# MacPhobos/audio-ident

Measured on AMD Instinct MI355X. Metric: audio-seconds fingerprinted/sec/GPU; landmark-hash bit-exact vs CPU ref, higher is better.
Workload: dtype f32; 1 GPU; BASELINE configs[1]: 256 x 10 s 44.1 kHz mono clips, fingerprint extraction per GPU; clips_per_gpu=256, n_fft=2048, hop=512, parallelism=clip-sharded x1 (no data-path collective)

## Files before the change

audio-ident_amd/csrc/aidfp_extract.h:

```cpp
#pragma once
#include "aidfp_buffers.h"
#include "aidfp_extract_plan.h"

namespace aid {

struct Extractor {
    DevBuf<float> pcm_stage, power;
    DevBuf<uint64_t> mask, hotw;
    DevBuf<uint32_t> clip_qmax;
    DevBuf<uint32_t> k2_cold;
    HostBuf<uint64_t> h_cold;
    uint64_t *h_cold_dev = nullptr;
    DevBuf<int64_t> chunk_counts, counts;
    DevBuf<uint64_t> records;
    DevBuf<ClipDesc> desc;
    HostBuf<ClipDesc> h_desc;
    size_t desc_n = 0;
    ClipDesc *desc_dev = nullptr;
    Event desc_ev, stage_ev;
    hipStream_t stage_stream = nullptr;
    K2Policy k2;
    int64_t k2_slots[2] = {1, 1};
    int64_t k1_slots = 1;
    int64_t plane_rows = 0;
    ExtractPlan plan;
    bool have_result = false;
};

}
```

audio-ident_amd/csrc/aidfp_extract_plan.h:

```cpp
#pragma once
#include <string.h>

#include <algorithm>
#include <vector>

#include "../../include/aidfp.h"
#include "aidfp_layout.h"

namespace aid {

constexpr int64_t kPlaneRows = (int64_t)3 << 18;
constexpr int kK2Hold = 64;

struct K2Choice {
    int width;
    double slots_x;
};

struct K2Policy {
    int width = 4;
    int hold = 0;
    int force_width = 0;
    double force_slots_x = 0.0;

    K2Choice choose(uint64_t cw, uint64_t sw) {
        const int seen_width = (sw >> 32) ? (int)((cw >> 32) / (sw >> 32)) : 0;
        if (force_width) {
            width = force_width;
        } else if (width == 4) {
            if (hold > 0) --hold;
            else if (seen_width == 4 && 2 * (uint64_t)(uint32_t)cw >= (cw >> 32)) width = 2;
        } else if (seen_width == 2 && (uint32_t)sw > 0) {
            width = 4;
            hold = kK2Hold;
        }
        if (force_slots_x > 0.0) return {width, force_slots_x};
        if (width != 4 || seen_width != 4) return {width, 1.0};
        const double c = std::min(1.0, (double)(uint32_t)cw / (double)(cw >> 32));
        return {width, c >= 0.45 ? 1.5 : c >= 0.3 ? 1.25 : 1.0};
    }
};

struct ClipGroup {
    int first = 0, n = 0;
    int64_t frame0 = 0, frames = 0;
    int64_t strips = 0, k1_strips = 0;
    int strip_len = 0;
};

struct ExtractPlan {
    std::vector<ClipDesc> desc;
    std::vector<int64_t> frames, hash_base;
    std::vector<ClipGroup> groups;
    int n_clips = 0, width = 4;
    int64_t total_frames = 0, strips = 0, chunks = 0, records = 0;
    int64_t staged = 0;
    bool empty_clip = false;
    bool multi_chunk = false, one_chunk_each = false;
};

inline void plan_extract(ExtractPlan &p, const int64_t *offsets, const int64_t *ends, int n_clips, int loc, int hop,
                         int64_t plane_rows, bool keep_power, int64_t slots, double slots_x, int width) {
    auto clip_end = [&](int c) { return ends ? ends[c] : offsets[c + 1]; };
    p.n_clips = n_clips;
    p.width = width;
    p.desc.resize(n_clips);
    p.frames.resize(n_clips);
    p.hash_base.resize(n_clips);
    p.groups.clear();
    const int64_t cap = plane_rows > 0 ? plane_rows : kPlaneRows;
    int first = 0;
    int64_t acc = 0;
    for (int c = 0; c < n_clips; ++c) {
        p.frames[c] = num_frames(clip_end(c) - offsets[c], hop);
        if (!keep_power && acc > 0 && acc + p.frames[c] > cap) {
            p.groups.push_back({first, c - first});
            first = c;
            acc = 0;
        }
        acc += p.frames[c];
    }
    p.groups.push_back({first, n_clips - first});
    p.total_frames = p.strips = p.chunks = p.records = 0;
    p.staged = loc == AID_PCM_HOST && n_clips > 0 ? clip_end(n_clips - 1) - offsets[0] : 0;
    p.empty_clip = p.multi_chunk = false;
    p.one_chunk_each = n_clips > 0;
    int64_t k1_strips = 0;
    for (ClipGroup &g : p.groups) {
        g.strip_len = peak_strip_len(p.frames.data() + g.first, g.n, std::max<int64_t>(1, (int64_t)(slots * slots_x)));
        g.frame0 = p.total_frames;
        for (int c = g.first; c < g.first + g.n; ++c) {
            const int64_t F = p.frames[c], nck = (F + kHashChunk - 1) / kHashChunk;
            p.desc[c] = {loc == AID_PCM_DEVICE ? offsets[c] : offsets[c] - offsets[0], F, p.total_frames, g.strips,
                         p.chunks, p.records, hash_capacity(F), k1_strips};
            p.hash_base[c] = p.records;
            p.empty_clip |= F == 0;
            p.multi_chunk |= nck > 1;
            p.one_chunk_each &= nck == 1;
            p.total_frames += F;
            g.frames += F;
            g.strips += (F + g.strip_len - 1) / g.strip_len;
            g.k1_strips += (F + kStftStrip - 1) / kStftStrip;
            k1_strips += (F + kStftStrip - 1) / kStftStrip;
            p.chunks += nck;
            p.records += hash_capacity(F);
        }
        p.strips += g.strips;
    }
}

inline bool desc_differ(const ClipDesc *a, size_t na, const ClipDesc *b, size_t nb) {
    return na != nb || (na > 0 && memcmp(a, b, na * sizeof(ClipDesc)) != 0);
}

}
```

audio-ident_amd/csrc/aidfp_launch.h:

```cpp
#pragma once
#include <hip/hip_runtime.h>
#include <stdint.h>

#include "aidfp_device.h"

namespace aid {
void launch_stft_power(const void *pcm, bool s16, const ClipDesc *clips, int n_clips, int64_t f0, int64_t total_frames,
                       int64_t total_strips, int64_t slots, int hop, const Tables *tab, float *out, bool logmag,
                       uint64_t *hot, float thr, bool keep_power, uint32_t *qmax, hipStream_t s);
int peak_pick_blocks_per_cu(int width);
void launch_peak_pick(int width, const float *power, const ClipDesc *clips, int n_clips, int64_t f0, int64_t total_strips,
                      int strip_len, float thr, const uint64_t *hot, uint64_t *mask, uint32_t *cold_cnt,
                      const uint32_t *clip_qmax, float rel, hipStream_t s);
void launch_landmarks(const uint64_t *mask, const ClipDesc *clips, int n_clips, int64_t total_chunks,
                      int64_t *chunk_counts, uint64_t *records, int64_t *clip_counts, bool write, uint32_t *k2_cold,
                      uint64_t *k2_cold_host, uint32_t k2_waves, uint32_t k2_strips, bool one_chunk_each,
                      hipStream_t s);
void launch_synth(float *out, const uint32_t *tracks, const int64_t *starts, int n_clips, int64_t n, int sr,
                  int noise_a, uint32_t salt, int fmax_hz, bool envelope, const int16_t *sin_tab, hipStream_t s);
void launch_resample(const void *src, bool s16, int64_t in_base, int64_t n, int channels, int up, int down, int hl,
                     int J, const float *taps, float *dst, int64_t m_first, int64_t count, hipStream_t s,
                     int n_streams = 1, int64_t src_stride = 0, int64_t dst_stride = 0, const void *hist = nullptr,
                     int64_t hist_n = 0, int64_t hist_stride = 0);
struct SpeedVarDev;
void launch_resample_speeds(const void *src, bool s16, int channels, const int64_t *clip_off, const SpeedVarDev *vars,
                            int n_speeds, const int64_t *blk_first, const int64_t *dst_off, int pair0, int n_pairs,
                            int64_t blocks, int64_t lds_floats, float *dst, hipStream_t s);
void launch_s16_to_f32(const int16_t *src, int64_t n, float *dst, hipStream_t s);
int dedup_chunks(int64_t n_cat);
void launch_dedup_scan(const uint32_t *cw, const int64_t *coff, const double *cdur, int64_t n_cat, const uint32_t *qw,
                       const int64_t *qoff, const double *qlo, const double *qhi, int nq, double *part_sim,
                       int64_t *part_idx, double *best_sim, int64_t *best_idx, hipStream_t s);
void launch_dedup_pairs(const uint32_t *aw, const int64_t *aoff, const uint32_t *bw, const int64_t *boff, int n,
                        double *sim, hipStream_t s);
void launch_index_count(const uint32_t *ph, const uint32_t *ptrack, int64_t n, const uint8_t *tomb, uint32_t n_tracks,
                        uint32_t *cnt, hipStream_t s);
void launch_index_scatter(const uint32_t *ph, const uint32_t *ptrack, const uint32_t *pt, int64_t n,
                          const uint8_t *tomb, uint32_t n_tracks, uint32_t *cursor, uint64_t *post, hipStream_t s);
void launch_scan(const uint32_t *in, uint32_t *out, int64_t n, uint32_t *tmp, hipStream_t s);
int match_lds_blocks_per_cu();
size_t radix_scratch_u32(int64_t n);
hipError_t launch_index_sort_build(const uint32_t *ph, const uint32_t *ptrack, const uint32_t *pt, int64_t n,
                                   const uint8_t *tomb, uint32_t n_tracks, uint32_t *keys0, uint32_t *keys1,
                                   uint64_t *vals0, uint64_t *vals1, uint32_t *scratch, uint32_t *E, uint32_t *offsets,
                                   unsigned long long *nz, uint64_t **vals_out, uint16_t *sig, int rank_mode,
                                   hipStream_t s);
void launch_make_sig(const uint64_t *post, int64_t n, uint16_t *sig, hipStream_t s);
void launch_compact(const uint32_t *ph, const uint32_t *ptrack, const uint32_t *pt, int64_t n, const uint8_t *tomb,
                    uint32_t n_tracks, uint32_t *cnt, uint32_t *off, uint32_t *tmp, uint32_t *oh, uint32_t *otrack,
                    uint32_t *ot, hipStream_t s);
// ... 45 lines not shown
```

audio-ident_amd/csrc/aidfp_layout.h:

```cpp
#pragma once
#include <stdint.h>

namespace aid {

constexpr int kN = 2048;
constexpr int kBins = 1024;
constexpr int kPeakDT = 7;
constexpr int kPeakDF = 15;
constexpr int kZoneDT = 63;
constexpr int kZoneDF = 127;
constexpr int kFan = 10;
constexpr int kMaskWords = kBins / 64;

constexpr int kStftWaves = 16;
constexpr int kStftStrip = 16;
constexpr int kK1MinFrames = 2;
constexpr int kStftLdsPerWave = 1092;

constexpr int kPeakStripMin = 16;
constexpr int kPeakStripMax = 65536;

inline int peak_strip_len(const int64_t *frames, int n, int64_t slots) {
    int64_t fmax = 0;
    for (int c = 0; c < n; ++c) fmax = frames[c] > fmax ? frames[c] : fmax;
// ... 2 lines not shown
        for (int c = 0; c < n; ++c) k += (frames[c] + L - 1) / L;
        return k;
    };
    int64_t lo = kPeakStripMin, hi = fmax > lo ? fmax : lo;
    if (hi > kPeakStripMax) hi = kPeakStripMax;
    if (count(lo) <= slots) return (int)lo;
    while (lo < hi) {
        const int64_t mid = (lo + hi) / 2;
        if (count(mid) <= slots) hi = mid; else lo = mid + 1;
    }
    return (int)lo;
}

constexpr int hot_bit(int c) { return c < 32 ? c : 95 - c; }

__host__ __device__ constexpr uint32_t bucket_key(uint32_t h) {
    return (((h >> 22) & 0xFFu) << 18) | ((h >> 30) << 16) | (((h >> 12) & 0x7Fu) << 9) | (((h >> 19) & 0x7u) << 6) |
           (h & 0x3Fu);
}

__host__ __device__ constexpr uint16_t posting_sig(uint32_t track, uint32_t t) {
    return (uint16_t)(((track * 0x9E3779B1u) >> 16) + t);
}

constexpr int64_t kLdsMaxVotes = (int64_t)1 << 18;

constexpr int kHashChunk = 1024;
constexpr int kHashChunkPeakCap = 64 * ((kHashChunk + kZoneDT + 7) / 8);

inline int64_t num_frames(int64_t n, int hop) { return (hop <= 0 || n < kN) ? 0 : 1 + (n - kN) / hop; }
inline int64_t peak_capacity(int64_t F) { return 64 * ((F + 7) / 8); }
inline int64_t hash_capacity(int64_t F) { return kFan * peak_capacity(F); }

struct ClipDesc {
    int64_t pcm_off;
    int64_t frames;
    int64_t frame_base;
    int64_t strip_base;
    int64_t chunk_base;
    int64_t hash_base;
    int64_t hash_cap;
    int64_t stft_base;
};

}
```

audio-ident_amd/csrc/extract.cpp:

```cpp
#include <cstring>

#include "engine_internal.h"

int extract_locked(aid_engine *e, const void *pcm, PcmFmt fmt, const int64_t *offsets, int32_t n_clips, int32_t loc,
                   void *stream, const int64_t *ends) {
    if (ends && loc != AID_PCM_DEVICE) return fail(AID_ERR_INVALID, "extract: clip ends need device PCM");
    HIP_TRY(hipSetDevice(e->device));
    Extractor &x = e->ext;
    ExtractPlan &p = x.plan;
    hipStream_t s = pick_stream(e, stream);
    const bool keep_power = (e->cfg.flags & AID_FLAG_KEEP_POWER) != 0, rel = e->cfg.peak_rel > 0.0f;
    if (e->last_stream && e->last_stream != s) HIP_TRY(hipStreamSynchronize(e->last_stream));
    x.have_result = false;
    const uint64_t cw = x.h_cold.p ? *reinterpret_cast<volatile uint64_t *>(x.h_cold.p) : 0;
    const uint64_t sw = x.h_cold.p ? *reinterpret_cast<volatile uint64_t *>(x.h_cold.p + 1) : 0;
    const K2Choice k2 = x.k2.choose(cw, sw);
    plan_extract(p, offsets, ends, n_clips, loc, e->cfg.hop, x.plane_rows, keep_power,
                 x.k2_slots[k2.width == 2 ? 0 : 1], k2.slots_x, k2.width);
    int64_t plane = 1;
    for (const ClipGroup &g : p.groups) plane = std::max(plane, g.frames);
    HIP_TRY(x.desc.reserve((size_t)n_clips + 1));
    HIP_TRY(x.power.reserve((size_t)plane * kBins));
    HIP_TRY(x.mask.reserve((size_t)p.total_frames * kMaskWords));
    HIP_TRY(x.hotw.reserve((size_t)p.total_frames + 1));
    if (rel) {
        HIP_TRY(x.clip_qmax.reserve((size_t)n_clips + 1));
        if (n_clips > 0) HIP_TRY(hipMemsetAsync(x.clip_qmax.p, 0, sizeof(uint32_t) * (size_t)n_clips, s));
    }
    if (!x.h_cold.p) {
        HIP_TRY(x.k2_cold.reserve(128));
        HIP_TRY(hipMemsetAsync(x.k2_cold.p, 0, 128 * sizeof(uint32_t), s));
        HIP_TRY(x.h_cold.reserve(2, hipHostMallocMapped));
        x.h_cold.p[0] = x.h_cold.p[1] = 0;
        HIP_TRY(hipHostGetDevicePointer((void **)&x.h_cold_dev, x.h_cold.p, 0));
    }
    HIP_TRY(x.chunk_counts.reserve((size_t)p.chunks + 1));
    HIP_TRY(x.records.reserve((size_t)p.records + 1));
    HIP_TRY(x.counts.reserve((size_t)n_clips + 1));
    const void *dpcm = pcm;
    if (p.staged > 0) {
        if (x.stage_stream != s) HIP_TRY(x.stage_ev.wait());
        x.stage_ev.live = false;
        const size_t nbytes = (size_t)p.staged * pcm_size(fmt);
        HIP_TRY(x.pcm_stage.reserve((nbytes + sizeof(float) - 1) / sizeof(float)));
        HIP_TRY(hipMemcpyAsync(x.pcm_stage.p, pcm_at(pcm, fmt, offsets[0]), nbytes, hipMemcpyHostToDevice, s));
        dpcm = x.pcm_stage.p;
    }
    if (n_clips > 0 && (x.desc_dev != x.desc.p || desc_differ(p.desc.data(), (size_t)n_clips, x.h_desc.p, x.desc_n))) {
        x.desc_dev = nullptr;
        HIP_TRY(x.desc_ev.wait());
        HIP_TRY(x.h_desc.reserve((size_t)n_clips + 1));
        std::memcpy(x.h_desc.p, p.desc.data(), sizeof(ClipDesc) * n_clips);
        HIP_TRY(hipMemcpyAsync(x.desc.p, x.h_desc.p, sizeof(ClipDesc) * n_clips, hipMemcpyHostToDevice, s));
        HIP_TRY(x.desc_ev.record(s));
        x.desc_n = (size_t)n_clips;
        x.desc_dev = x.desc.p;
    }
    if (p.empty_clip || p.total_frames == 0)
        HIP_TRY(hipMemsetAsync(x.counts.p, 0, sizeof(int64_t) * ((size_t)n_clips + 1), s));
    if (p.total_frames > 0) {
        for (const ClipGroup &g : p.groups) {
            if (g.frames == 0) continue;
            uint32_t *qmax = rel ? x.clip_qmax.p + g.first : nullptr;
            {
                ProfScope ps(e, AID_K_STFT, s, true);
                launch_stft_power(dpcm, fmt == kS16, x.desc.p + g.first, g.n, g.frame0, g.frames, g.k1_strips,
                                  x.k1_slots, e->cfg.hop, e->d_tab.p, x.power.p, false, x.hotw.p,
                                  e->cfg.peak_threshold, keep_power, qmax, s);
            }
            if (loc == AID_PCM_HOST && &g == &p.groups.back()) {
                HIP_TRY(x.stage_ev.record(s));
                x.stage_stream = s;
            }
            {
                ProfScope ps(e, AID_K_PEAKS, s, true);
                launch_peak_pick(p.width, x.power.p, x.desc.p + g.first, g.n, g.frame0, g.strips, g.strip_len,
                                 e->cfg.peak_threshold, x.hotw.p, x.mask.p, x.k2_cold.p, qmax, e->cfg.peak_rel, s);
            }
        }
        if (p.multi_chunk) {
            ProfScope ps(e, AID_K_LANDMARK_COUNT, s, true);
            launch_landmarks(x.mask.p, x.desc.p, n_clips, p.chunks, x.chunk_counts.p, x.records.p, x.counts.p, false,
                             nullptr, nullptr, 0u, 0u, p.one_chunk_each, s);
        }
        {
            ProfScope ps(e, AID_K_LANDMARK_WRITE, s, true);
            launch_landmarks(x.mask.p, x.desc.p, n_clips, p.chunks, x.chunk_counts.p, x.records.p, x.counts.p, true,
                             x.h_cold_dev ? x.k2_cold.p : nullptr, x.h_cold_dev, (uint32_t)(p.width * p.strips),
                             (uint32_t)p.strips, p.one_chunk_each, s);
        }
    }
    HIP_TRY(hipGetLastError());
    e->last_stream = s;
    x.have_result = true;
    return AID_OK;
}

static int result_ready(aid_engine *e, const int32_t *clip, bool wait = true) {
    if (!e) return fail(AID_ERR_INVALID, "null engine");
    if (!e->ext.have_result) return fail(AID_ERR_STATE, "no extraction yet");
    if (clip && (*clip < 0 || *clip >= e->ext.plan.n_clips)) return fail(AID_ERR_INVALID, "clip index out of range");
    return wait ? aid_sync(e) : AID_OK;
}

template <typename T>
static int read_rows(aid_engine *e, int32_t clip, const T *plane, int per, T *out, int64_t cap) {
    const ClipDesc &d = e->ext.plan.desc[clip];
    if (d.frames * per > cap) return fail(AID_ERR_INVALID, "output capacity too small");
    if (d.frames > 0)
        HIP_TRY(hipMemcpy(out, plane + d.frame_base * per, d.frames * per * sizeof(T), hipMemcpyDeviceToHost));
    return AID_OK;
}

extern "C" {

int64_t aid_num_frames(const aid_engine *e, int64_t n) { return e ? num_frames(n, e->cfg.hop) : 0; }
int64_t aid_hash_capacity(const aid_engine *e, int64_t n) { return e ? hash_capacity(num_frames(n, e->cfg.hop)) : 0; }

static int extract_entry(const char *fn, aid_engine *e, const void *pcm, PcmFmt fmt, const int64_t *offsets,
                         int32_t n_clips, int32_t loc, void *stream) {
    if (int rc = check_clips(fn, e, pcm, offsets, n_clips, loc)) return rc;
    std::lock_guard<std::mutex> lk(e->mu);
// ... 44 lines not shown
    if (counts_dev) *counts_dev = e->ext.counts.p;
    if (clip_base_host) *clip_base_host = e->ext.plan.hash_base.data();
    if (n_clips) *n_clips = e->ext.plan.n_clips;
    return AID_OK;
}

int aid_result_power(aid_engine *e, int32_t clip, float *out, int64_t cap) {
    if (int rc = result_ready(e, &clip)) return rc;
    if (!(e->cfg.flags & AID_FLAG_KEEP_POWER))
        return fail(AID_ERR_STATE, "aid_result_power: engine created without AID_FLAG_KEEP_POWER (cold blocks not stored)");
    if (int rc = read_rows(e, clip, e->ext.power.p, kBins, out, cap)) return rc;
    for (int64_t i = 0; i < e->ext.plan.frames[clip] * kBins; ++i) out[i] = out[i] * 0.25f;
    return AID_OK;
}

int aid_result_thresholds(aid_engine *e, float *out) {
    if (int rc = result_ready(e, nullptr)) return rc;
    const int n = e->ext.plan.n_clips;
    if (n > 0 && !out) return fail(AID_ERR_INVALID, "null argument");
    const float thr = e->cfg.peak_threshold, r = e->cfg.peak_rel;
    std::vector<uint32_t> q((size_t)n, 0u);
    if (r > 0.0f && n > 0) HIP_TRY(hipMemcpy(q.data(), e->ext.clip_qmax.p, sizeof(uint32_t) * n, hipMemcpyDeviceToHost));
    for (int c = 0; c < n; ++c) {
        float qm;
        std::memcpy(&qm, &q[c], sizeof(qm));
        const float t = r * (qm * 0.25f);
        out[c] = t > thr ? t : thr;
    }
    return AID_OK;
}

int aid_result_peakmask(aid_engine *e, int32_t clip, uint64_t *out, int64_t cap) {
    if (int rc = result_ready(e, &clip)) return rc;
    return read_rows(e, clip, e->ext.mask.p, kMaskWords, out, cap);
}

int aid_spectrogram(aid_engine *e, const float *pcm, int64_t n, float *out, int64_t cap) {
    if (!e || (n > 0 && !pcm) || n < 0) return fail(AID_ERR_INVALID, "aid_spectrogram: bad argument");
    const int64_t F = num_frames(n, e->cfg.hop);
    if (F * kBins > cap) return fail(AID_ERR_INVALID, "output capacity too small");
    if (F == 0) return AID_OK;
    EngineCall call(e, nullptr, false, kDrainLast);
    if (call.rc) return call.rc;
    hipStream_t s = call.s;
    DevBuf<float> d_pcm, d_out;
    DevBuf<ClipDesc> d_desc;
    ClipDesc d{};
    d.frames = F;
    HIP_TRY(d_pcm.reserve((size_t)n));
    hipError_t he = d_out.reserve((size_t)(F * kBins));
    if (he == hipSuccess) he = d_desc.reserve(1);
    if (he == hipSuccess) he = hipMemcpy(d_pcm.p, pcm, n * sizeof(float), hipMemcpyHostToDevice);
    if (he == hipSuccess) he = hipMemcpy(d_desc.p, &d, sizeof(ClipDesc), hipMemcpyHostToDevice);
    if (he == hipSuccess)
        launch_stft_power(d_pcm.p, false, d_desc.p, 1, 0, F, (F + kStftStrip - 1) / kStftStrip, e->ext.k1_slots,
                          e->cfg.hop, e->d_tab.p, d_out.p, true, nullptr, e->cfg.peak_threshold, true, nullptr, s);
    if (he == hipSuccess) he = hipGetLastError();
    if (he == hipSuccess) he = hipStreamSynchronize(s);
    if (he == hipSuccess) he = hipMemcpy(out, d_out.p, F * kBins * sizeof(float), hipMemcpyDeviceToHost);
    return he == hipSuccess ? AID_OK : fail(AID_ERR_DEVICE, std::string("aid_spectrogram: ") + hipGetErrorString(he));
}

}
```

audio-ident_amd/csrc/landmarks.hip:

```cpp
#include "aidfp_device.h"
#include "aidfp_launch.h"

namespace aid {

constexpr int kK3 = 512;

__device__ __forceinline__ int64_t block_excl_scan(int64_t v, int64_t *tmp , int64_t *total) {
    const int tid = threadIdx.x, lane = tid & 63, w = tid >> 6;
    int64_t x = v;
#pragma unroll
    for (int off = 1; off < 64; off <<= 1) {
        const int64_t y = __shfl_up(x, off, 64);
        if (lane >= off) x += y;
    }
    if (lane == 63) tmp[w] = x;
    __syncthreads();
    int64_t base = 0, tot = 0;
#pragma unroll
    for (int i = 0; i < kK3 / 64; ++i) {
        const int64_t t = tmp[i];
        base += i < w ? t : 0;
        tot += t;
    }
    if (total) *total = tot;
    __syncthreads();
    return base + x - v;
}

__device__ __forceinline__ uint32_t make_hash(int k1, int k2, int dt) {
    return ((uint32_t)(k1 & 0x3FF) << 22) | ((uint32_t)(k2 & 0x3FF) << 12) | ((uint32_t)dt & 0xFFF);
}

template <bool WRITE>
__global__ __launch_bounds__(kK3) void k_landmarks(const uint64_t *__restrict__ mask, const ClipDesc *__restrict__ clips,
                                                  int n_clips, int64_t total_chunks, int64_t *__restrict__ chunk_counts,
                                                  uint64_t *__restrict__ records, int64_t *__restrict__ clip_counts,
                                                  uint32_t *__restrict__ k2_cold, uint64_t *__restrict__ k2_cold_host,
                                                  uint32_t k2_waves, uint32_t k2_strips, int one_chunk_each) {
    __shared__ uint32_t plist[kHashChunkPeakCap];
    __shared__ uint32_t foff[kHashChunk + kZoneDT + 2];
    __shared__ int64_t scan_tmp[kK3];
    const int tid = threadIdx.x;
    const int64_t chunk = blockIdx.x;
    if (WRITE && k2_cold && blockIdx.x == 0 && tid < 64) {
        uint32_t c = k2_cold[tid], c2 = k2_cold[64 + tid];
        k2_cold[tid] = 0u;
        k2_cold[64 + tid] = 0u;
        for (int o = 32; o > 0; o >>= 1) {
            c += __shfl_xor(c, o);
            c2 += __shfl_xor(c2, o);
        }
        if (tid == 0) {
            volatile uint64_t *h = reinterpret_cast<volatile uint64_t *>(k2_cold_host);
            h[0] = (uint64_t)c | ((uint64_t)k2_waves << 32);
            h[1] = (uint64_t)c2 | ((uint64_t)k2_strips << 32);
        }
    }
    if (chunk >= total_chunks) return;
    int lo = 0, hi = n_clips - 1;
    if (one_chunk_each) lo = (int)chunk;
    while (lo < hi) {
        const int mid = (lo + hi + 1) >> 1;
        if (clips[mid].chunk_base <= chunk) lo = mid; else hi = mid - 1;
    }
    const ClipDesc cd = clips[lo];
    const int64_t F = cd.frames;
    const int64_t q = chunk - cd.chunk_base;
    const int64_t c0 = q * kHashChunk;
    const int64_t c1 = min(c0 + (int64_t)kHashChunk, F);
    const int64_t g1 = min(c1 + (int64_t)kZoneDT, F);
    const int nf = (int)(g1 - c0);
    const uint64_t *Mc = mask + (cd.frame_base + c0) * kMaskWords;
    const int64_t nck = (F + kHashChunk - 1) / kHashChunk;
    if (!WRITE && nck == 1) return;

    const int per = (nf + kK3 - 1) / kK3;
    const int fa = min(tid * per, nf), fz = min(fa + per, nf);
    int64_t mine = 0;
    for (int f = fa; f < fz; ++f) {
        uint32_t c = 0;
#pragma unroll
        for (int w = 0; w < kMaskWords; ++w) c += __popcll(Mc[f * kMaskWords + w]);
        foff[f] = c;
        mine += c;
    }
    int64_t npk = 0;
    int64_t run = block_excl_scan(mine, scan_tmp, &npk);
    for (int f = fa; f < fz; ++f) {
        const uint32_t c = foff[f];
        foff[f] = (uint32_t)run;
        if (c == 0) continue;
        int64_t idx = run;
        uint64_t W[kMaskWords];
#pragma unroll
        for (int w = 0; w < kMaskWords; ++w) W[w] = Mc[f * kMaskWords + w];
#pragma unroll
        for (int b = 0; b < 4; ++b) {
            const uint64_t w1 = W[4 * b + 1], w2 = W[4 * b + 2], w3 = W[4 * b + 3];
            for (uint64_t m = W[4 * b] | w1 | w2 | w3; m; m &= m - 1) {
                const int l = __ffsll((unsigned long long)m) - 1;
                const int i = (int)((w1 >> l) & 1) + 2 * (int)((w2 >> l) & 1) + 3 * (int)((w3 >> l) & 1);
                plist[idx++] = ((uint32_t)f << 10) | (uint32_t)(256 * b + 4 * l + i);
            }
        }
        run += c;
    }
    if (tid == 0) foff[nf] = (uint32_t)npk;
    __syncthreads();
    const int n_anchor = (int)foff[c1 - c0];

    const int pa_per = (n_anchor + kK3 - 1) / kK3;
    const int aa = min(tid * pa_per, n_anchor), az = min(aa + pa_per, n_anchor);
    int64_t my = 0;
    uint64_t tmask = 0;
    bool tmask_ok = false;
    for (int i = aa; i < az; ++i) {
        const uint32_t a = plist[i];
        const int ta = (int)(a >> 10), ka = (int)(a & 1023);
        int got = 0;
        uint64_t mk = 0;
        bool ok = true;
        for (int j = i + 1; j < (int)npk && got < kFan; ++j) {
            const uint32_t b = plist[j];
            const int dt = (int)(b >> 10) - ta;
            if (dt > kZoneDT) break;
            if (dt <= 0) continue;
            const int df = (int)(b & 1023) - ka;
            if (df < -kZoneDF || df > kZoneDF) continue;
            if (j - i - 1 < 64) mk |= 1ull << (j - i - 1);
            else ok = false;
            ++got;
        }
// ... 22 lines not shown
                block_excl_scan(all, scan_tmp, &tot);
                if (tid == 0) clip_counts[lo] = tot;
            }
        }
        uint64_t *out = records + cd.hash_base + before + excl;
        int64_t o = 0;
        for (int i = aa; i < az; ++i) {
            const uint32_t a = plist[i];
            const int ta = (int)(a >> 10), ka = (int)(a & 1023);
            const uint64_t t1 = (uint64_t)(c0 + ta) << 32;
            if (i == aa && tmask_ok) {
                for (uint64_t m = tmask; m; m &= m - 1) {
                    const uint32_t b = plist[i + 1 + (__ffsll((unsigned long long)m) - 1)];
                    out[o++] = t1 | make_hash(ka, (int)(b & 1023), (int)(b >> 10) - ta);
                }
                continue;
            }
            int got = 0;
            for (int j = i + 1; j < (int)npk && got < kFan; ++j) {
                const uint32_t b = plist[j];
                const int dt = (int)(b >> 10) - ta;
                if (dt > kZoneDT) break;
                if (dt <= 0) continue;
                const int kb = (int)(b & 1023);
                const int df = kb - ka;
                if (df < -kZoneDF || df > kZoneDF) continue;
                out[o++] = t1 | make_hash(ka, kb, dt);
                ++got;
            }
        }
    }
}

void launch_landmarks(const uint64_t *mask, const ClipDesc *clips, int n_clips, int64_t total_chunks,
                      int64_t *chunk_counts, uint64_t *records, int64_t *clip_counts, bool write, uint32_t *k2_cold,
                      uint64_t *k2_cold_host, uint32_t k2_waves, uint32_t k2_strips, bool one_chunk_each,
                      hipStream_t s) {
    if (total_chunks <= 0) return;
    if (write)
        timed_launch(k_landmarks<true>, dim3((unsigned)total_chunks), dim3(kK3), 0, s, mask, clips, n_clips,
                           total_chunks, chunk_counts, records, clip_counts, k2_cold, k2_cold_host, k2_waves,
                     k2_strips, one_chunk_each ? 1 : 0);
    else
        timed_launch(k_landmarks<false>, dim3((unsigned)total_chunks), dim3(kK3), 0, s, mask, clips, n_clips,
                           total_chunks, chunk_counts, records, clip_counts, (uint32_t *)nullptr, (uint64_t *)nullptr, 0u,
                     0u, one_chunk_each ? 1 : 0);
}

}
```

audio-ident_amd/csrc/peaks.hip:

```cpp
#include "aidfp_device.h"
#include "aidfp_launch.h"

namespace aid {

constexpr int kRowsPerStep = 4;

#if defined(AID_K2_STAMPS)
__device__ unsigned long long g_k2_stamps[8];
#define AID_K2_T() ((unsigned long long)__builtin_amdgcn_s_memtime())
#endif

template <int LANE>
__device__ __forceinline__ uint32_t write_lane(uint32_t v, uint32_t s_val) {
    asm volatile("v_writelane_b32 %0, %1, %2" : "+v"(v) : "s"(s_val), "i"(LANE));
    return v;
}

__device__ __forceinline__ int pkey(float x) {
    float r;
    asm("v_max_f32 %0, 0, %1" : "=v"(r) : "v"(x));
    return __float_as_int(r);
}

struct PeakPickArgs {
    const float *power;
    const ClipDesc *clips;
    int n_clips;
    int64_t f0, total_strips;
    int strip_len;
    float thr;
    const uint64_t *hot;
    uint64_t *mask;
    uint32_t *cold_cnt;
    const uint32_t *clip_qmax;
    float rel;
};

template <int W>
#if defined(AID_K2_PF2) && defined(AID_K2_OCC3)
__global__ __launch_bounds__(64 * W, 3) void k_peak_pick(
#else
__global__ __launch_bounds__(64 * W, 4) void k_peak_pick(
#endif
                                                  const float *__restrict__ power_, const ClipDesc *__restrict__ clips_,
                                                  int n_clips_, int64_t f0_, int64_t total_strips_, int strip_len_, float thr_,
                                                  const uint64_t *__restrict__ hot_, uint64_t *__restrict__ mask_,
                                                  uint32_t *__restrict__ cold_cnt_,
                                                  const uint32_t *__restrict__ clip_qmax_, float rel_) {
    static_assert(W == 2 || W == 4, "quarter waves per workgroup");
    constexpr int kGB = 256 * W;
    __shared__ __attribute__((aligned(16))) int rows[kRowsPerStep][kGB + 32];
    __shared__ __attribute__((aligned(16))) int bms[kRowsPerStep][64 * W + 8];
#pragma unroll
    for (int g = 0; g < 4 / W; ++g) {
        const float *power = power_;
        const ClipDesc *clips = clips_;
        int n_clips = n_clips_, strip_len = strip_len_;
        int64_t f0 = f0_, total_strips = total_strips_;
        float thr = thr_, rel = rel_;
        const uint64_t *hot = hot_;
        uint64_t *mask = mask_;
        uint32_t *cold_cnt = cold_cnt_;
        const uint32_t *clip_qmax = clip_qmax_;
        if (g > 0) {
            typedef const __attribute__((address_space(4))) PeakPickArgs *ArgPtr;
            ArgPtr a = (ArgPtr)__builtin_amdgcn_kernarg_segment_ptr();
            asm volatile("" : "+s"(a));
            power = a->power, clips = a->clips, n_clips = a->n_clips, f0 = a->f0, total_strips = a->total_strips;
            strip_len = a->strip_len, thr = a->thr, hot = a->hot, mask = a->mask, cold_cnt = a->cold_cnt;
            clip_qmax = a->clip_qmax, rel = a->rel;
            __syncthreads();
        }
#if defined(AID_K2_STAMPS)
        const unsigned long long st_birth = AID_K2_T();
        unsigned long long st_bar = 0, st_b0 = 0, st_b1 = 0;
#endif
        const int lane = threadIdx.x & 63;
        const int wl = __builtin_amdgcn_readfirstlane(((int)(threadIdx.x >> 6) + (int)blockIdx.x) & (W - 1));
        const int wave = wl + W * g;
        const int tid = wave * 64 + lane;
        const int lt = wl * 64 + lane;
        constexpr int kInf = 0x7F800000;

        int64_t strip;
        {
            const int64_t nb = gridDim.x, b = blockIdx.x;
            const int64_t per = nb / 8, rem = nb % 8, x = b % 8, y = b / 8;
            strip = (x < rem ? x * (per + 1) : rem * (per + 1) + (x - rem) * per) + y;
            strip = nb - 1 - strip;
        }
        if (strip >= total_strips) return;
        int lo = 0, hi = n_clips - 1;
        while (lo < hi) {
            const int mid = (lo + hi + 1) >> 1;
            if (clips[mid].strip_base <= strip) lo = mid; else hi = mid - 1;
        }
        const int F = (int)clips[lo].frames;
        const int64_t fb = clips[lo].frame_base;
        const int t0 = (int)(strip - clips[lo].strip_base) * strip_len;
        const int t1 = min(t0 + strip_len, F);
        const float *P = power + (fb - f0) * kBins;
        uint64_t *M = mask + fb * kMaskWords + 4 * wave + lane;
        int kthr = __float_as_int(4.0f * thr);
        if (clip_qmax) kthr = max(kthr, __float_as_int(rel * __uint_as_float(clip_qmax[lo])));

        const int rbeg = t0 - kPeakDT;
        const int iters = (t1 - t0) + 2 * kPeakDT;
        const uint64_t *HW = hot + fb;
        auto hotword = [&](int r) -> uint64_t { return (r >= 0 && r < F) ? HW[r] : 0ull; };
        auto hotwords = [&](int rb) -> uint64_t {
            const int r = rb + (lane & 3);
            return (r >= 0 && r < F) ? HW[r] : 0ull;
        };
        auto word_of = [](uint64_t v, int j) -> uint64_t {
            return ((uint64_t)(uint32_t)__builtin_amdgcn_readlane((int)(v >> 32), j) << 32) |
                   (uint32_t)__builtin_amdgcn_readlane((int)v, j);
        };

        const int bwl = g == 0 ? W - 1 : 0;

        if constexpr (W == 4) {
            if (tid < 16) {
#pragma unroll
                for (int r = 0; r < kRowsPerStep; ++r) {
                    rows[r][tid] = 0;
                    rows[r][kBins + 16 + tid] = 0;
                    if (tid < 4) {
                        bms[r][tid] = 0;
                        bms[r][260 + tid] = 0;
                    }
                }
            }
        } else if (lane < 16) {
#pragma unroll
            for (int r = 0; r < kRowsPerStep; ++r) {
// ... 4 lines not shown
                if (wl == W - 1) {
                    rows[r][kGB + 16 + lane] = 0;
                    if (lane < 4) bms[r][64 * W + 4 + lane] = 0;
                }
            }
        }

        int m2r[8][4];
        int pend[8][4];
        int fprev[4], m7p[4];
#pragma unroll
        for (int s = 0; s < 8; ++s)
#pragma unroll
            for (int i = 0; i < 4; ++i) { m2r[s][i] = 0; pend[s][i] = -1; }
#pragma unroll
        for (int i = 0; i < 4; ++i) { fprev[i] = 0; m7p[i] = 0; }
        const uint64_t b0ok = __ballot(tid != 0);

        const int myb = hot_bit(tid >> 2);
        uint64_t wmask = 0;
        for (int c = max(16 * wave - 1, 0); c <= min(16 * wave + 16, 63); ++c) wmask |= 1ull << hot_bit(c);
        bool need2 = false, bhot = false;
        {
            uint64_t acc = 0;
            for (int r = rbeg + lane; r < rbeg + iters; r += 64) acc |= (r >= 0 && r < F) ? HW[r] : 0ull;
            bool cold = __ballot((acc & wmask) != 0ull) == 0;
            if (W < 4) {
                bhot = __ballot((acc >> hot_bit(g == 0 ? 16 * W : 16 * W - 1)) & 1ull) != 0;
                if (g == 0) {
                    uint64_t up = 0;
                    for (int c = 16 * W - 1; c < 64; ++c) up |= 1ull << hot_bit(c);
                    need2 = __ballot((acc & up) != 0ull) != 0;
                    if (!need2) {
                        uint64_t *Mz = mask + fb * kMaskWords + 4 * (W + wl) + (lane & 3);
                        for (int r = t0 + (lane >> 2); r < t1; r += 16) Mz[(int64_t)r * kMaskWords] = 0;
                    } else {
                        cold = false;
                        if (wl == 0 && lane == 0 && cold_cnt) atomicAdd(&cold_cnt[64 + (blockIdx.x & 63)], 1u);
                    }
                }
            }
            if (cold) {
#pragma unroll
                for (int j = 0; j < kRowsPerStep; ++j) {
                    reinterpret_cast<int4 *>(&rows[j][16])[lt] = make_int4(0, 0, 0, 0);
                    bms[j][4 + lt] = 0;
                }
                uint64_t *Mz = mask + fb * kMaskWords + 4 * wave + (lane & 3);
                for (int r = t0 + (lane >> 2); r < t1; r += 16) Mz[(int64_t)r * kMaskWords] = 0;
                if (lane == 0 && cold_cnt && g == 0) atomicAdd(&cold_cnt[blockIdx.x & 63], 1u);
#if defined(AID_K2_STAMPS)
                if (lane == 0) atomicAdd(&g_k2_stamps[7], 1ull);
#endif
                asm volatile("s_waitcnt lgkmcnt(0)" ::: "memory");
                return;
            }
        }
        const int rlo = max(rbeg, 0), rhi = min(rbeg + iters, F);
        constexpr uint32_t kOOB = 0x80000000u;
        const __amdgpu_buffer_rsrc_t rows_rsrc = __builtin_amdgcn_make_buffer_rsrc(
            const_cast<float *>(P + (int64_t)rlo * kBins), (short)0, (rhi - rlo) * kBins * 4, 0x00020000);
        auto load_row = [&](int r, uint64_t hwr) -> float4 {
            const uint32_t off = ((hwr >> myb) & 1ull) ? (uint32_t)(r - rlo) * (kBins * 4) + 16u * tid : kOOB;
            const auto v = __builtin_amdgcn_raw_buffer_load_b128(rows_rsrc, off, 0, 0);
            return make_float4(__int_as_float(v[0]), __int_as_float(v[1]), __int_as_float(v[2]), __int_as_float(v[3]));
        };
#if defined(AID_K2_PF2)
        float4 pfb[2][kRowsPerStep];
        uint64_t hs[2][kRowsPerStep], hcur[kRowsPerStep];
#pragma unroll
        for (int b = 0; b < 2; ++b)
#pragma unroll
            for (int j = 0; j < kRowsPerStep; ++j) {
                const int r = rbeg + b * kRowsPerStep + j;
                hs[b][j] = hotword(r);
                pfb[b][j] = load_row(r, b * kRowsPerStep + j < iters ? hs[b][j] : 0ull);
                hcur[j] = 0ull;
            }
        uint64_t hwv = hotwords(rbeg + 2 * kRowsPerStep);
#else
        float4 pf[kRowsPerStep];
#pragma unroll
        for (int j = 0; j < kRowsPerStep; ++j) pf[j] = load_row(rbeg + j, j < iters ? hotword(rbeg + j) : 0ull);
        uint64_t hwv = hotwords(rbeg + kRowsPerStep);
        uint64_t hsave[kRowsPerStep], hcur[kRowsPerStep];
#pragma unroll
        for (int j = 0; j < kRowsPerStep; ++j) hsave[j] = hcur[j] = hotword(rbeg + j);
#endif

        for (int base = 0; base < iters; base += 8) {
#pragma unroll
            for (int s = 0; s < 8; ++s) {
                const int it = base + s;
                if (it >= iters) break;
                if (s % kRowsPerStep == 0) {
#if defined(AID_K2_STAMPS)
                    st_bar += st_b1 - st_b0;
                    st_b0 = AID_K2_T();
                    if (it > 0) __syncthreads();
                    st_b1 = AID_K2_T();
#else
                    if (it > 0) __syncthreads();
#endif
#if defined(AID_K2_PF2)
                    const int b = (s / kRowsPerStep) & 1;
#pragma unroll
                    for (int j = 0; j < kRowsPerStep; ++j) {
                        const float4 v = pfb[b][j];
                        const int4 kv = make_int4(pkey(v.x), pkey(v.y), pkey(v.z), pkey(v.w));
                        reinterpret_cast<int4 *>(&rows[j][16])[lt] = kv;
                        bms[j][4 + lt] = max(max(kv.x, kv.y), max(kv.z, kv.w));
                        const int rn = rbeg + it + j + 2 * kRowsPerStep;
                        hcur[j] = hs[b][j];
                        hs[b][j] = word_of(hwv, j);
                        pfb[b][j] = load_row(rn, it + j + 2 * kRowsPerStep < iters ? hs[b][j] : 0ull);
                    }
                    hwv = hotwords(rbeg + it + 3 * kRowsPerStep);
#else
#pragma unroll
                    for (int j = 0; j < kRowsPerStep; ++j) {
                        const int slot = (s + j) % kRowsPerStep;
                        const float4 v = pf[slot];
// ... 53 lines not shown
                const int mpre1 = max(me.x, me.y), mpre2 = max(mpre1, me.z);
                const int msuf2 = max(me.z, me.w), msuf1 = max(me.y, msuf2);
                int L[4], R[4];
                L[0] = max(lsuf1, M3L);
                L[1] = max(max(lsuf2, M3L), me.x);
                L[2] = max(max(lf.w, M3L), mpre1);
                L[3] = max(M3L, mpre2);
                R[0] = max(msuf1, M3R);
                R[1] = max(max(msuf2, M3R), rt.x);
                R[2] = max(max(me.w, M3R), rpre1);
                R[3] = max(M3R, rpre2);
                const int mev[4] = {me.x, me.y, me.z, me.w};

                const int thr_row = (r >= t0 && r < t1) ? kthr : kInf;
#pragma unroll
                for (int i = 0; i < 4; ++i) {
                    const int p = mev[i];
                    const int fm = max(max(L[i], p), R[i]);
                    const int m2 = max(fm, fprev[i]);
                    fprev[i] = fm;
                    const int bf = max(max(L[i], thr_row), m7p[i]);
                    m2r[s][i] = m2;
                    const int m7 = max(max(max(m2, m2r[(s - 2) & 7][i]), m2r[(s - 4) & 7][i]), m2r[(s - 5) & 7][i]);
                    m7p[i] = m7;
                    pk[i] = pend[(s + 1) & 7][i] >= m7;
                    bal[i] = __ballot(pk[i]);
                    bool cand = p > bf && p >= R[i];
                    if (i == 0) cand = cand && ((b0ok >> lane) & 1ull);
                    pend[s][i] = cand ? p : -1;
                }
                }
                const uint64_t b0 = bal[0], b1 = bal[1], b2 = bal[2], b3 = bal[3];
                const int rd = r - kPeakDT;
                if (rd >= t0 && rd < t1) {
                    uint32_t lo, hi;
                    asm volatile("" : "=v"(lo), "=v"(hi));
                    lo = write_lane<0>(lo, (uint32_t)b0);
                    hi = write_lane<0>(hi, (uint32_t)(b0 >> 32));
                    lo = write_lane<1>(lo, (uint32_t)b1);
                    hi = write_lane<1>(hi, (uint32_t)(b1 >> 32));
                    lo = write_lane<2>(lo, (uint32_t)b2);
                    hi = write_lane<2>(hi, (uint32_t)(b2 >> 32));
                    lo = write_lane<3>(lo, (uint32_t)b3);
                    hi = write_lane<3>(hi, (uint32_t)(b3 >> 32));
                    if (lane < 4) M[(int64_t)rd * kMaskWords] = ((uint64_t)hi << 32) | lo;
                }
            }
        }
#if defined(AID_K2_STAMPS)
        {
            const unsigned long long t = AID_K2_T();
            st_bar += st_b1 - st_b0;
            if (lane == 0) {
                atomicAdd(&g_k2_stamps[0], st_bar);
                atomicAdd(&g_k2_stamps[5], 1ull);
                atomicAdd(&g_k2_stamps[6], t - st_birth);
            }
        }
#endif
        if (!need2) break;
    }
}

#if defined(AID_K2_STAMPS)
int k2_stamps_read(unsigned long long *out, bool reset) {
    if (hipMemcpyFromSymbol(out, HIP_SYMBOL(g_k2_stamps), sizeof(unsigned long long) * 8) != hipSuccess) return -2;
    if (reset) {
        const unsigned long long z[8] = {};
        if (hipMemcpyToSymbol(HIP_SYMBOL(g_k2_stamps), z, sizeof(z)) != hipSuccess) return -2;
    }
    return 0;
}
#endif

void launch_peak_pick(int width, const float *power, const ClipDesc *clips, int n_clips, int64_t f0, int64_t total_strips,
                      int strip_len, float thr, const uint64_t *hot, uint64_t *mask, uint32_t *cold_cnt,
                      const uint32_t *clip_qmax, float rel, hipStream_t s) {
    if (total_strips <= 0) return;
    if (width == 2)
        timed_launch(k_peak_pick<2>, dim3((unsigned)total_strips), dim3(128), 0, s, power, clips, n_clips, f0,
                     total_strips, strip_len, thr, hot, mask, cold_cnt, clip_qmax, rel);
    else
        timed_launch(k_peak_pick<4>, dim3((unsigned)total_strips), dim3(256), 0, s, power, clips, n_clips, f0,
                     total_strips, strip_len, thr, hot, mask, cold_cnt, clip_qmax, rel);
}

int peak_pick_blocks_per_cu(int width) {
    int n = 0;
    const hipError_t rc = width == 2 ? hipOccupancyMaxActiveBlocksPerMultiprocessor(&n, k_peak_pick<2>, 128, 0)
                                     : hipOccupancyMaxActiveBlocksPerMultiprocessor(&n, k_peak_pick<4>, 256, 0);
    if (rc != hipSuccess || n <= 0) n = 1;
    return n;
}

}
```

Before: 6.725 million audio-s/s.

## Emit per-row peak flags and skip zero mask writes and reads

Peak picking now writes a mask row only when it holds a peak, and records a compact per-row, per-quarter bitmap of non-empty rows in a new rowflags buffer. Cold quarters clear only their flag words instead of zeroing mask rows. The landmark kernel reads these flags to skip popcounts and loads of empty mask rows, and the host peakmask readback applies the flags to zero stale rows. This cuts mask write and read traffic, at the cost of an extra buffer, more indexing and stale data left in the mask buffer.

```diff
diff --git a/audio-ident_amd/csrc/aidfp_extract.h b/audio-ident_amd/csrc/aidfp_extract.h
--- a/audio-ident_amd/csrc/aidfp_extract.h
+++ b/audio-ident_amd/csrc/aidfp_extract.h
@@ -7,6 +7,7 @@
 struct Extractor {
     DevBuf<float> pcm_stage, power;
     DevBuf<uint64_t> mask, hotw;
+    DevBuf<uint32_t> rowflags;
     DevBuf<uint32_t> clip_qmax;
     DevBuf<uint32_t> k2_cold;
     HostBuf<uint64_t> h_cold;
diff --git a/audio-ident_amd/csrc/aidfp_extract_plan.h b/audio-ident_amd/csrc/aidfp_extract_plan.h
--- a/audio-ident_amd/csrc/aidfp_extract_plan.h
+++ b/audio-ident_amd/csrc/aidfp_extract_plan.h
@@ -46,6 +46,7 @@
     int64_t frame0 = 0, frames = 0;
     int64_t strips = 0, k1_strips = 0;
     int strip_len = 0;
+    int64_t flag_base = 0;
 };
 
 struct ExtractPlan {
@@ -53,7 +54,7 @@
     std::vector<int64_t> frames, hash_base;
     std::vector<ClipGroup> groups;
     int n_clips = 0, width = 4;
-    int64_t total_frames = 0, strips = 0, chunks = 0, records = 0;
+    int64_t total_frames = 0, strips = 0, chunks = 0, records = 0, flag_words = 0;
     int64_t staged = 0;
     bool empty_clip = false;
     bool multi_chunk = false, one_chunk_each = false;
@@ -81,7 +82,7 @@
         acc += p.frames[c];
     }
     p.groups.push_back({first, n_clips - first});
-    p.total_frames = p.strips = p.chunks = p.records = 0;
+    p.total_frames = p.strips = p.chunks = p.records = p.flag_words = 0;
     p.staged = loc == AID_PCM_HOST && n_clips > 0 ? clip_end(n_clips - 1) - offsets[0] : 0;
     p.empty_clip = p.multi_chunk = false;
     p.one_chunk_each = n_clips > 0;
@@ -89,10 +90,12 @@
     for (ClipGroup &g : p.groups) {
         g.strip_len = peak_strip_len(p.frames.data() + g.first, g.n, std::max<int64_t>(1, (int64_t)(slots * slots_x)));
         g.frame0 = p.total_frames;
+        g.flag_base = p.flag_words;
         for (int c = g.first; c < g.first + g.n; ++c) {
             const int64_t F = p.frames[c], nck = (F + kHashChunk - 1) / kHashChunk;
             p.desc[c] = {loc == AID_PCM_DEVICE ? offsets[c] : offsets[c] - offsets[0], F, p.total_frames, g.strips,
-                         p.chunks, p.records, hash_capacity(F), k1_strips};
+                         p.chunks, p.records, hash_capacity(F), k1_strips,
+                         g.flag_base + g.strips * flag_words_per_strip(g.strip_len), g.strip_len};
             p.hash_base[c] = p.records;
             p.empty_clip |= F == 0;
             p.multi_chunk |= nck > 1;
@@ -106,6 +109,7 @@
             p.records += hash_capacity(F);
         }
         p.strips += g.strips;
+        p.flag_words += g.strips * flag_words_per_strip(g.strip_len);
     }
 }
 
diff --git a/audio-ident_amd/csrc/aidfp_launch.h b/audio-ident_amd/csrc/aidfp_launch.h
--- a/audio-ident_amd/csrc/aidfp_launch.h
+++ b/audio-ident_amd/csrc/aidfp_launch.h
@@ -11,11 +11,11 @@
 int peak_pick_blocks_per_cu(int width);
 void launch_peak_pick(int width, const float *power, const ClipDesc *clips, int n_clips, int64_t f0, int64_t total_strips,
                       int strip_len, float thr, const uint64_t *hot, uint64_t *mask, uint32_t *cold_cnt,
-                      const uint32_t *clip_qmax, float rel, hipStream_t s);
-void launch_landmarks(const uint64_t *mask, const ClipDesc *clips, int n_clips, int64_t total_chunks,
-                      int64_t *chunk_counts, uint64_t *records, int64_t *clip_counts, bool write, uint32_t *k2_cold,
-                      uint64_t *k2_cold_host, uint32_t k2_waves, uint32_t k2_strips, bool one_chunk_each,
-                      hipStream_t s);
+                      const uint32_t *clip_qmax, float rel, uint32_t *rowflags, hipStream_t s);
+void launch_landmarks(const uint64_t *mask, const uint32_t *rowflags, const ClipDesc *clips, int n_clips,
+                      int64_t total_chunks, int64_t *chunk_counts, uint64_t *records, int64_t *clip_counts, bool write,
+                      uint32_t *k2_cold, uint64_t *k2_cold_host, uint32_t k2_waves, uint32_t k2_strips,
+                      bool one_chunk_each, hipStream_t s);
 void launch_synth(float *out, const uint32_t *tracks, const int64_t *starts, int n_clips, int64_t n, int sr,
                   int noise_a, uint32_t salt, int fmax_hz, bool envelope, const int16_t *sin_tab, hipStream_t s);
 void launch_resample(const void *src, bool s16, int64_t in_base, int64_t n, int channels, int up, int down, int hl,
diff --git a/audio-ident_amd/csrc/aidfp_layout.h b/audio-ident_amd/csrc/aidfp_layout.h
--- a/audio-ident_amd/csrc/aidfp_layout.h
+++ b/audio-ident_amd/csrc/aidfp_layout.h
@@ -58,6 +58,8 @@
 inline int64_t peak_capacity(int64_t F) { return 64 * ((F + 7) / 8); }
 inline int64_t hash_capacity(int64_t F) { return kFan * peak_capacity(F); }
 
+constexpr int64_t flag_words_per_strip(int strip_len) { return 4 * (((int64_t)strip_len + 31) / 32); }
+
 struct ClipDesc {
     int64_t pcm_off;
     int64_t frames;
@@ -67,6 +69,8 @@
     int64_t hash_base;
     int64_t hash_cap;
     int64_t stft_base;
+    int64_t flag_base;
+    int64_t strip_len;
 };
 
 }
diff --git a/audio-ident_amd/csrc/extract.cpp b/audio-ident_amd/csrc/extract.cpp
--- a/audio-ident_amd/csrc/extract.cpp
+++ b/audio-ident_amd/csrc/extract.cpp
@@ -22,6 +22,7 @@
     HIP_TRY(x.desc.reserve((size_t)n_clips + 1));
     HIP_TRY(x.power.reserve((size_t)plane * kBins));
     HIP_TRY(x.mask.reserve((size_t)p.total_frames * kMaskWords));
+    HIP_TRY(x.rowflags.reserve((size_t)p.flag_words + 4));
     HIP_TRY(x.hotw.reserve((size_t)p.total_frames + 1));
     if (rel) {
         HIP_TRY(x.clip_qmax.reserve((size_t)n_clips + 1));
@@ -75,19 +76,20 @@
             {
                 ProfScope ps(e, AID_K_PEAKS, s, true);
                 launch_peak_pick(p.width, x.power.p, x.desc.p + g.first, g.n, g.frame0, g.strips, g.strip_len,
-                                 e->cfg.peak_threshold, x.hotw.p, x.mask.p, x.k2_cold.p, qmax, e->cfg.peak_rel, s);
+                                 e->cfg.peak_threshold, x.hotw.p, x.mask.p, x.k2_cold.p, qmax, e->cfg.peak_rel,
+                                 x.rowflags.p, s);
             }
         }
         if (p.multi_chunk) {
             ProfScope ps(e, AID_K_LANDMARK_COUNT, s, true);
-            launch_landmarks(x.mask.p, x.desc.p, n_clips, p.chunks, x.chunk_counts.p, x.records.p, x.counts.p, false,
-                             nullptr, nullptr, 0u, 0u, p.one_chunk_each, s);
+            launch_landmarks(x.mask.p, x.rowflags.p, x.desc.p, n_clips, p.chunks, x.chunk_counts.p, x.records.p,
+                             x.counts.p, false, nullptr, nullptr, 0u, 0u, p.one_chunk_each, s);
         }
         {
             ProfScope ps(e, AID_K_LANDMARK_WRITE, s, true);
-            launch_landmarks(x.mask.p, x.desc.p, n_clips, p.chunks, x.chunk_counts.p, x.records.p, x.counts.p, true,
-                             x.h_cold_dev ? x.k2_cold.p : nullptr, x.h_cold_dev, (uint32_t)(p.width * p.strips),
-                             (uint32_t)p.strips, p.one_chunk_each, s);
+            launch_landmarks(x.mask.p, x.rowflags.p, x.desc.p, n_clips, p.chunks, x.chunk_counts.p, x.records.p,
+                             x.counts.p, true, x.h_cold_dev ? x.k2_cold.p : nullptr, x.h_cold_dev,
+                             (uint32_t)(p.width * p.strips), (uint32_t)p.strips, p.one_chunk_each, s);
         }
     }
     HIP_TRY(hipGetLastError());
@@ -198,7 +200,19 @@
 
 int aid_result_peakmask(aid_engine *e, int32_t clip, uint64_t *out, int64_t cap) {
     if (int rc = result_ready(e, &clip)) return rc;
-    return read_rows(e, clip, e->ext.mask.p, kMaskWords, out, cap);
+    if (int rc = read_rows(e, clip, e->ext.mask.p, kMaskWords, out, cap)) return rc;
+    const ClipDesc &d = e->ext.plan.desc[clip];
+    if (d.frames == 0) return AID_OK;
+    const int64_t L = d.strip_len, per = flag_words_per_strip((int)L);
+    std::vector<uint32_t> fl((size_t)(((d.frames + L - 1) / L) * per));
+    HIP_TRY(hipMemcpy(fl.data(), e->ext.rowflags.p + d.flag_base, fl.size() * sizeof(uint32_t), hipMemcpyDeviceToHost));
+    for (int64_t r = 0; r < d.frames; ++r) {
+        const int64_t o = r % L;
+        const uint32_t *unit = fl.data() + (r / L) * per + 4 * (o >> 5);
+        for (int q = 0; q < 4; ++q)
+            if (!((unit[q] >> (o & 31)) & 1u)) std::memset(out + r * kMaskWords + 4 * q, 0, 4 * sizeof(uint64_t));
+    }
+    return AID_OK;
 }
 
 int aid_spectrogram(aid_engine *e, const float *pcm, int64_t n, float *out, int64_t cap) {
diff --git a/audio-ident_amd/csrc/landmarks.hip b/audio-ident_amd/csrc/landmarks.hip
--- a/audio-ident_amd/csrc/landmarks.hip
+++ b/audio-ident_amd/csrc/landmarks.hip
@@ -32,8 +32,10 @@
 }
 
 template <bool WRITE>
-__global__ __launch_bounds__(kK3) void k_landmarks(const uint64_t *__restrict__ mask, const ClipDesc *__restrict__ clips,
-                                                  int n_clips, int64_t total_chunks, int64_t *__restrict__ chunk_counts,
+__global__ __launch_bounds__(kK3) void k_landmarks(const uint64_t *__restrict__ mask,
+                                                  const uint32_t *__restrict__ rowflags,
+                                                  const ClipDesc *__restrict__ clips, int n_clips,
+                                                  int64_t total_chunks, int64_t *__restrict__ chunk_counts,
                                                   uint64_t *__restrict__ records, int64_t *__restrict__ clip_counts,
                                                   uint32_t *__restrict__ k2_cold, uint64_t *__restrict__ k2_cold_host,
                                                   uint32_t k2_waves, uint32_t k2_strips, int one_chunk_each) {
@@ -77,27 +79,50 @@
     const int per = (nf + kK3 - 1) / kK3;
     const int fa = min(tid * per, nf), fz = min(fa + per, nf);
     int64_t mine = 0;
-    for (int f = fa; f < fz; ++f) {
+    const uint32_t L = (uint32_t)cd.strip_len;
+    const uint32_t *FLc = rowflags + cd.flag_base;
+    const int64_t fnw = flag_words_per_strip((int)L);
+    constexpr int kP1 = (kHashChunk + kZoneDT + kK3 - 1) / kK3;
+    uint32_t nibs[kP1];
+#pragma unroll
+    for (int i = 0; i < kP1; ++i) {
+        const int f = tid + i * kK3;
+        nibs[i] = 0;
+        if (f < nf) {
+            const uint32_t fr = (uint32_t)(c0 + f), st = fr / L, o = fr - st * L;
+            const uint4 fu = *reinterpret_cast<const uint4 *>(FLc + st * fnw + 4 * (o >> 5));
+            nibs[i] = ((fu.x >> (o & 31)) & 1u) | ((fu.y >> (o & 31)) & 1u) << 1 | ((fu.z >> (o & 31)) & 1u) << 2 |
+                      ((fu.w >> (o & 31)) & 1u) << 3;
+        }
+    }
+#pragma unroll
+    for (int i = 0; i < kP1; ++i) {
+        const int f = tid + i * kK3;
+        if (f >= nf) continue;
         uint32_t c = 0;
 #pragma unroll
-        for (int w = 0; w < kMaskWords; ++w) c += __popcll(Mc[f * kMaskWords + w]);
-        foff[f] = c;
-        mine += c;
-    }
+        for (int b = 0; b < 4; ++b) {
+            if (!((nibs[i] >> b) & 1u)) continue;
+#pragma unroll
+            for (int w = 4 * b; w < 4 * b + 4; ++w) c += __popcll(Mc[f * kMaskWords + w]);
+        }
+        foff[f] = c | nibs[i] << 28;
+    }
+    __syncthreads();
+    for (int f = fa; f < fz; ++f) mine += foff[f] & 0x0FFFFFFFu;
     int64_t npk = 0;
     int64_t run = block_excl_scan(mine, scan_tmp, &npk);
     for (int f = fa; f < fz; ++f) {
-        const uint32_t c = foff[f];
+        const uint32_t c = foff[f] & 0x0FFFFFFFu, nib = foff[f] >> 28;
         foff[f] = (uint32_t)run;
         if (c == 0) continue;
         int64_t idx = run;
-        uint64_t W[kMaskWords];
-#pragma unroll
-        for (int w = 0; w < kMaskWords; ++w) W[w] = Mc[f * kMaskWords + w];
 #pragma unroll
         for (int b = 0; b < 4; ++b) {
-            const uint64_t w1 = W[4 * b + 1], w2 = W[4 * b + 2], w3 = W[4 * b + 3];
-            for (uint64_t m = W[4 * b] | w1 | w2 | w3; m; m &= m - 1) {
+            if (!((nib >> b) & 1u)) continue;
+            const uint64_t *Wb = Mc + f * kMaskWords + 4 * b;
+            const uint64_t w0 = Wb[0], w1 = Wb[1], w2 = Wb[2], w3 = Wb[3];
+            for (uint64_t m = w0 | w1 | w2 | w3; m; m &= m - 1) {
                 const int l = __ffsll((unsigned long long)m) - 1;
                 const int i = (int)((w1 >> l) & 1) + 2 * (int)((w2 >> l) & 1) + 3 * (int)((w3 >> l) & 1);
                 plist[idx++] = ((uint32_t)f << 10) | (uint32_t)(256 * b + 4 * l + i);
@@ -186,17 +211,17 @@
     }
 }
 
-void launch_landmarks(const uint64_t *mask, const ClipDesc *clips, int n_clips, int64_t total_chunks,
-                      int64_t *chunk_counts, uint64_t *records, int64_t *clip_counts, bool write, uint32_t *k2_cold,
-                      uint64_t *k2_cold_host, uint32_t k2_waves, uint32_t k2_strips, bool one_chunk_each,
-                      hipStream_t s) {
+void launch_landmarks(const uint64_t *mask, const uint32_t *rowflags, const ClipDesc *clips, int n_clips,
+                      int64_t total_chunks, int64_t *chunk_counts, uint64_t *records, int64_t *clip_counts, bool write,
+                      uint32_t *k2_cold, uint64_t *k2_cold_host, uint32_t k2_waves, uint32_t k2_strips,
+                      bool one_chunk_each, hipStream_t s) {
     if (total_chunks <= 0) return;
     if (write)
-        timed_launch(k_landmarks<true>, dim3((unsigned)total_chunks), dim3(kK3), 0, s, mask, clips, n_clips,
+        timed_launch(k_landmarks<true>, dim3((unsigned)total_chunks), dim3(kK3), 0, s, mask, rowflags, clips, n_clips,
                            total_chunks, chunk_counts, records, clip_counts, k2_cold, k2_cold_host, k2_waves,
                      k2_strips, one_chunk_each ? 1 : 0);
     else
-        timed_launch(k_landmarks<false>, dim3((unsigned)total_chunks), dim3(kK3), 0, s, mask, clips, n_clips,
+        timed_launch(k_landmarks<false>, dim3((unsigned)total_chunks), dim3(kK3), 0, s, mask, rowflags, clips, n_clips,
                            total_chunks, chunk_counts, records, clip_counts, (uint32_t *)nullptr, (uint64_t *)nullptr, 0u,
                      0u, one_chunk_each ? 1 : 0);
 }
diff --git a/audio-ident_amd/csrc/peaks.hip b/audio-ident_amd/csrc/peaks.hip
--- a/audio-ident_amd/csrc/peaks.hip
+++ b/audio-ident_amd/csrc/peaks.hip
@@ -34,6 +34,7 @@
     uint32_t *cold_cnt;
     const uint32_t *clip_qmax;
     float rel;
+    uint32_t *rowflags;
 };
 
 template <int W>
@@ -46,7 +47,8 @@
                                                   int n_clips_, int64_t f0_, int64_t total_strips_, int strip_len_, float thr_,
                                                   const uint64_t *__restrict__ hot_, uint64_t *__restrict__ mask_,
                                                   uint32_t *__restrict__ cold_cnt_,
-                                                  const uint32_t *__restrict__ clip_qmax_, float rel_) {
+                                                  const uint32_t *__restrict__ clip_qmax_, float rel_,
+                                                  uint32_t *__restrict__ rowflags_) {
     static_assert(W == 2 || W == 4, "quarter waves per workgroup");
     constexpr int kGB = 256 * W;
     __shared__ __attribute__((aligned(16))) int rows[kRowsPerStep][kGB + 32];
@@ -62,13 +64,14 @@
         uint64_t *mask = mask_;
         uint32_t *cold_cnt = cold_cnt_;
         const uint32_t *clip_qmax = clip_qmax_;
+        uint32_t *rowflags = rowflags_;
         if (g > 0) {
             typedef const __attribute__((address_space(4))) PeakPickArgs *ArgPtr;
             ArgPtr a = (ArgPtr)__builtin_amdgcn_kernarg_segment_ptr();
             asm volatile("" : "+s"(a));
             power = a->power, clips = a->clips, n_clips = a->n_clips, f0 = a->f0, total_strips = a->total_strips;
             strip_len = a->strip_len, thr = a->thr, hot = a->hot, mask = a->mask, cold_cnt = a->cold_cnt;
-            clip_qmax = a->clip_qmax, rel = a->rel;
+            clip_qmax = a->clip_qmax, rel = a->rel, rowflags = a->rowflags;
             __syncthreads();
         }
 #if defined(AID_K2_STAMPS)
@@ -101,6 +104,15 @@
         const int t1 = min(t0 + strip_len, F);
         const float *P = power + (fb - f0) * kBins;
         uint64_t *M = mask + fb * kMaskWords + 4 * wave + lane;
+        const int nw = (strip_len + 31) >> 5;
+        uint32_t *FL = rowflags + clips[lo].flag_base + (strip - clips[lo].strip_base) * (4 * nw);
+        auto no_peaks = [&](int q) {
+#if defined(AID_K2_EMIT_ALL)
+            uint64_t *Mz = mask + fb * kMaskWords + 4 * q + (lane & 3);
+            for (int r = t0 + (lane >> 2); r < t1; r += 16) Mz[(int64_t)r * kMaskWords] = 0;
+#endif
+            for (int j = lane; j < nw; j += 64) FL[4 * j + q] = 0u;
+        };
         int kthr = __float_as_int(4.0f * thr);
         if (clip_qmax) kthr = max(kthr, __float_as_int(rel * __uint_as_float(clip_qmax[lo])));
 
@@ -171,8 +183,7 @@
                     for (int c = 16 * W - 1; c < 64; ++c) up |= 1ull << hot_bit(c);
                     need2 = __ballot((acc & up) != 0ull) != 0;
                     if (!need2) {
-                        uint64_t *Mz = mask + fb * kMaskWords + 4 * (W + wl) + (lane & 3);
-                        for (int r = t0 + (lane >> 2); r < t1; r += 16) Mz[(int64_t)r * kMaskWords] = 0;
+                        no_peaks(W + wl);
                     } else {
                         cold = false;
                         if (wl == 0 && lane == 0 && cold_cnt) atomicAdd(&cold_cnt[64 + (blockIdx.x & 63)], 1u);
@@ -185,8 +196,7 @@
                     reinterpret_cast<int4 *>(&rows[j][16])[lt] = make_int4(0, 0, 0, 0);
                     bms[j][4 + lt] = 0;
                 }
-                uint64_t *Mz = mask + fb * kMaskWords + 4 * wave + (lane & 3);
-                for (int r = t0 + (lane >> 2); r < t1; r += 16) Mz[(int64_t)r * kMaskWords] = 0;
+                no_peaks(wave);
                 if (lane == 0 && cold_cnt && g == 0) atomicAdd(&cold_cnt[blockIdx.x & 63], 1u);
 #if defined(AID_K2_STAMPS)
                 if (lane == 0) atomicAdd(&g_k2_stamps[7], 1ull);
@@ -227,6 +237,7 @@
         for (int j = 0; j < kRowsPerStep; ++j) hsave[j] = hcur[j] = hotword(rbeg + j);
 #endif
 
+        uint32_t fw = 0u;
         for (int base = 0; base < iters; base += 8) {
 #pragma unroll
             for (int s = 0; s < 8; ++s) {
@@ -346,7 +357,19 @@
                 }
                 const uint64_t b0 = bal[0], b1 = bal[1], b2 = bal[2], b3 = bal[3];
                 const int rd = r - kPeakDT;
-                if (rd >= t0 && rd < t1) {
+#if defined(AID_K2_NOEMIT)
+                asm volatile("" ::"s"(b0), "s"(b1), "s"(b2), "s"(b3));
+                const bool nz = false;
+#else
+                const uint64_t ball = b0 | b1 | b2 | b3;
+                const bool nz = ball != 0ull;
+                fw |= min((uint32_t)__builtin_popcountll(ball), 1u) << ((it - 2 * kPeakDT) & 31);
+#endif
+#if defined(AID_K2_EMIT_ALL)
+                if (it >= 2 * kPeakDT) {
+#else
+                if (nz) {
+#endif
                     uint32_t lo, hi;
                     asm volatile("" : "=v"(lo), "=v"(hi));
                     lo = write_lane<0>(lo, (uint32_t)b0);
@@ -359,7 +382,16 @@
                     hi = write_lane<3>(hi, (uint32_t)(b3 >> 32));
                     if (lane < 4) M[(int64_t)rd * kMaskWords] = ((uint64_t)hi << 32) | lo;
                 }
-            }
+                if (s == (2 * kPeakDT + 31) % 8 && it > 2 * kPeakDT && ((it - 2 * kPeakDT) & 31) == 31) {
+                    if (lane == 0) FL[((it - 2 * kPeakDT) >> 5) * 4 + wave] = fw;
+                    fw = 0u;
+                }
+            }
+        }
+        {
+            const int nr = t1 - t0;
+            if (lane == 0 && (nr & 31)) FL[(nr >> 5) * 4 + wave] = fw;
+            for (int j = ((nr + 31) >> 5) + lane; j < nw; j += 64) FL[4 * j + wave] = 0u;
         }
 #if defined(AID_K2_STAMPS)
         {
@@ -389,14 +421,14 @@
 
 void launch_peak_pick(int width, const float *power, const ClipDesc *clips, int n_clips, int64_t f0, int64_t total_strips,
                       int strip_len, float thr, const uint64_t *hot, uint64_t *mask, uint32_t *cold_cnt,
-                      const uint32_t *clip_qmax, float rel, hipStream_t s) {
+                      const uint32_t *clip_qmax, float rel, uint32_t *rowflags, hipStream_t s) {
     if (total_strips <= 0) return;
     if (width == 2)
         timed_launch(k_peak_pick<2>, dim3((unsigned)total_strips), dim3(128), 0, s, power, clips, n_clips, f0,
-                     total_strips, strip_len, thr, hot, mask, cold_cnt, clip_qmax, rel);
+                     total_strips, strip_len, thr, hot, mask, cold_cnt, clip_qmax, rel, rowflags);
     else
         timed_launch(k_peak_pick<4>, dim3((unsigned)total_strips), dim3(256), 0, s, power, clips, n_clips, f0,
-                     total_strips, strip_len, thr, hot, mask, cold_cnt, clip_qmax, rel);
+                     total_strips, strip_len, thr, hot, mask, cold_cnt, clip_qmax, rel, rowflags);
 }
 
 int peak_pick_blocks_per_cu(int width) {
```

After: 6.803 million audio-s/s (median of 6 runs). 1.01x the previous value.
